# Sudo42b/vision.cpp

Measured on AMD Instinct MI355X. Metric: images/sec, Depth-Anything-V2-Small 518x518 f16, higher is better.
Workload: dtype f16; 1 GPU; Depth-Anything-V2-Small f16 (DINOv2-S ViT) 518x518 batch=32 per MI355X (BASELINE.json configs[1]); global_batch=32, weights=random-init synthetic GGUF (seed 0), parallelism=dp1 (image shards, no data-path collective), hip_graph=True

## Files before the change

### vision.cpp_amd/csrc/kernels_attn.hip

```cpp
#include "vx_common.h"

#include <cstdlib>
#include <type_traits>

namespace {

#ifndef VISP_ATTN_WPE
#define VISP_ATTN_WPE 4
#endif
#ifndef VISP_ATTN_RS
#define VISP_ATTN_RS 1
#endif
#ifndef VISP_ATTN_SEQ
#define VISP_ATTN_SEQ 1
#endif
constexpr int HD = 64;
constexpr int KV_TILE = 64;
constexpr int Q_PER_WAVE = 32;
constexpr int TILE_BYTES = KV_TILE * HD * 2;
constexpr float FAST_LIMIT_DEFAULT = 1024.0f;

typedef __fp16 hv4 __attribute__((__vector_size__(4 * sizeof(__fp16))));

__device__ __forceinline__ int v_swz(int row, int chunk16) { return chunk16 ^ (((row >> 1) & 1) << 2); }

template <int NW, bool STAMP = false>
__global__ __launch_bounds__(64 * NW) __attribute__((amdgpu_waves_per_eu(VISP_ATTN_WPE, VISP_ATTN_WPE))) void attention_kernel(const f16* __restrict__ Q, const f16* __restrict__ K,
                                                         const f16* __restrict__ V, f16* __restrict__ O, int H, int T, float FAST_LIMIT,
                                                         unsigned long long* __restrict__ stamps = nullptr) {
    unsigned long long st_wait = 0, st_soft = 0, st_pv = 0, st_t0 = 0;
    if constexpr (STAMP) st_t0 = __builtin_amdgcn_s_memtime();
    __shared__ __attribute__((aligned(16))) unsigned char smem[2 * 2 * TILE_BYTES];

    const int tid = threadIdx.x, lane = tid & 63;
    const int wave = __builtin_amdgcn_readfirstlane(tid >> 6);
    const int r = lane & 31, h = lane >> 5;
    constexpr int Q_PER_BLOCK = Q_PER_WAVE * NW;
    const int n_qblk = (T + Q_PER_BLOCK - 1) / Q_PER_BLOCK;
    int logical;
    {
        const int total = gridDim.x, id = blockIdx.x;
        const int per = total >> 3, rem = total & 7, xcd = id & 7;
        logical = (xcd < rem ? xcd * (per + 1) : rem * (per + 1) + (xcd - rem) * per) + (id >> 3);
    }
    const int bh = logical / n_qblk;
    const int q0 = (logical - bh * n_qblk) * Q_PER_BLOCK + wave * Q_PER_WAVE;

    const f16* Qb = Q + (long)bh * T * HD;
    const f16* Kb = K + (long)bh * T * HD;
    const f16* Vb = V + (long)bh * T * HD;

    f16x8 qf[4];
    {
        int qrow = q0 + r;
        if (qrow >= T) qrow = T - 1;
#pragma unroll
        for (int s = 0; s < 4; ++s) qf[s] = *reinterpret_cast<const f16x8*>(Qb + (long)qrow * HD + 16 * s + 8 * h);
    }

    const int l_row = lane >> 3, l_pos = lane & 7;
    const int n_tiles = (T + KV_TILE - 1) / KV_TILE;
    const __amdgpu_buffer_rsrc_t k_rsrc = __builtin_amdgcn_make_buffer_rsrc(const_cast<f16*>(Kb), 0, T * HD * 2, 0x00020000);
    const __amdgpu_buffer_rsrc_t v_rsrc = __builtin_amdgcn_make_buffer_rsrc(const_cast<f16*>(Vb), 0, T * HD * 2, 0x00020000);

    auto issue_loads = [&](int t, int buf) {
        unsigned char* sk = smem + buf * (2 * TILE_BYTES);
        unsigned char* sv = sk + TILE_BYTES;
        const int tile_bytes0 = t * (KV_TILE * HD * 2);
        constexpr int PER = 8 / NW;
#pragma unroll
        for (int i = 0; i < PER; ++i) {
            const int piece = wave * PER + i, row = piece * 8 + l_row;
            __builtin_amdgcn_raw_ptr_buffer_load_lds(k_rsrc, (lptr_t)(sk + piece * 1024), 16,
                                                     tile_bytes0 + row * (HD * 2) + swz128(row, l_pos) * 16, 0, 0, 0);
            __builtin_amdgcn_raw_ptr_buffer_load_lds(v_rsrc, (lptr_t)(sv + piece * 1024), 16,
                                                     tile_bytes0 + row * (HD * 2) + v_swz(row, l_pos) * 16, 0, 0, 0);
        }
    };

    f32x16 o[2];
#pragma unroll
    for (int e = 0; e < 16; ++e) { o[0][e] = 0.0f; o[1][e] = 0.0f; }
    float m_run = 0.0f;
    float l_run = 0.0f;

    const int tr_q = (lane & 15) >> 2, tr_p = lane & 3, tr_d0 = 16 * ((lane >> 4) & 1);
    const int k_off0 = r * 128 + swz128(r, h) * 16;
    int v_off0;
    {
        const int key = 4 * h + tr_q, dd = tr_d0 + 4 * tr_p;
        v_off0 = key * 128 + v_swz(key, dd >> 3) * 16 + (dd & 7) * 2;
    }
    auto k_off = [&](int st) { return k_off0 ^ (st << 5); };
    auto v_off = [&](int db) { return v_off0 ^ (db << 6); };

    f32x16 negm;
#pragma unroll
    for (int e = 0; e < 16; ++e) negm[e] = 0.0f;

    auto qk = [&](const unsigned char* sk, int kb, int k0, bool masked) {
        f32x16 s;
#pragma unroll
        for (int st = 0; st < 4; ++st) {
            f16x8 kf = *reinterpret_cast<const f16x8*>(sk + k_off(st) + kb * 4096);
            s = __builtin_amdgcn_mfma_f32_32x32x16_f16(kf, qf[st], st == 0 ? negm : s, 0, 0, 0);
        }
        if (masked) {
#pragma unroll
            for (int e = 0; e < 16; ++e) {
                const int key = k0 + kb * 32 + (e & 3) + 8 * (e >> 2) + 4 * h;
                if (key >= T) s[e] = -INFINITY;
            }
        }
        return s;
    };
    const f16x8 ones = {(f16)1, (f16)1, (f16)1, (f16)1, (f16)1, (f16)1, (f16)1, (f16)1};
    auto softmax_p = [&](const unsigned char* sk, int k0, bool masked, f16x8 (&pf)[4]) {
#pragma unroll
        for (int kb = 0; kb < 2; ++kb) {
            f32x16 s = qk(sk, kb, k0, masked);
#pragma unroll
            for (int e = 0; e < 16; ++e) pf[2 * kb + (e >> 3)][e & 7] = (f16)__builtin_amdgcn_exp2f(s[e]);
            if (VISP_ATTN_SEQ) __builtin_amdgcn_sched_barrier(0);
        }
        if constexpr (VISP_ATTN_RS) {
            typedef _Float16 h2 __attribute__((ext_vector_type(2)));
            h2 t[16];
#pragma unroll
            for (int i = 0; i < 16; ++i) t[i] = h2{pf[i >> 2][2 * (i & 3)], pf[i >> 2][2 * (i & 3) + 1]};
#pragma unroll
            for (int w = 8; w >= (VISP_ATTN_RS == 2 ? 4 : 1); w >>= 1)
#pragma unroll
                for (int i = 0; i < w; ++i) t[i] = t[i] + t[i + w];
            float half_sum;
            if (VISP_ATTN_RS == 2)
                half_sum = (((float)t[0][0] + (float)t[0][1]) + ((float)t[1][0] + (float)t[1][1])) + (((float)t[2][0] + (float)t[2][1]) + ((float)t[3][0] + (float)t[3][1]));
            else
                half_sum = (float)t[0][0] + (float)t[0][1];
            return half_sum + other_half(half_sum);
        }
        f32x16 rs = {0.f, 0.f, 0.f, 0.f, 0.f, 0.f, 0.f, 0.f, 0.f, 0.f, 0.f, 0.f, 0.f, 0.f, 0.f, 0.f};
#pragma unroll
        for (int ks = 0; ks < 4; ++ks) rs = __builtin_amdgcn_mfma_f32_32x32x16_f16(ones, pf[ks], rs, 0, 0, 0);
        return rs[0];
    };
    auto pv = [&](const unsigned char* sv, const f16x8 (&pf)[4]) {
#pragma unroll
        for (int ks = 0; ks < 4; ++ks) {
#pragma unroll
            for (int db = 0; db < 2; ++db) {
                hv4 va = __builtin_amdgcn_ds_read_tr16_b64_v4f16(
                    (__attribute__((address_space(3))) hv4*)(sv + v_off(db) + ks * 2048));
                hv4 vb = __builtin_amdgcn_ds_read_tr16_b64_v4f16(
                    (__attribute__((address_space(3))) hv4*)(sv + v_off(db) + ks * 2048 + 1024));
                f16x8 vf = {(f16)va[0], (f16)va[1], (f16)va[2], (f16)va[3], (f16)vb[0], (f16)vb[1], (f16)vb[2], (f16)vb[3]};
                o[db] = __builtin_amdgcn_mfma_f32_32x32x16_f16(vf, pf[ks], o[db], 0, 0, 0);
            }
        }
    };

    auto tile_body = [&](int t, auto buf_c) {
        constexpr int BUF = decltype(buf_c)::value;
        unsigned long long c0 = 0, c1 = 0, c2 = 0;
        if constexpr (STAMP) c0 = __builtin_amdgcn_s_memtime();
        wait_vmcnt<0>();
        __syncthreads();
        if (t + 1 < n_tiles) issue_loads(t + 1, BUF ^ 1);
        if constexpr (STAMP) { c1 = __builtin_amdgcn_s_memtime(); st_wait += c1 - c0; }
        const unsigned char* sk = smem + BUF * (2 * TILE_BYTES);
        const unsigned char* sv = sk + TILE_BYTES;
        if (q0 >= T) return;
        const int k0 = t * KV_TILE;
        const bool last = k0 + KV_TILE > T;
        f16x8 pf[4];
        float psum = 0.0f;

        bool done = false;
        if (t > 0 && !last) {
            psum = softmax_p(sk, k0, false, pf);
            done = !__any(!(psum <= FAST_LIMIT));
        }
        if (!done) {
            float mloc = -INFINITY;
#pragma unroll
            for (int kb = 0; kb < 2; ++kb) {
                const f32x16 s = qk(sk, kb, k0, last);
#pragma unroll
                for (int e = 0; e < 16; ++e) mloc = fmaxf(mloc, s[e]);
                __builtin_amdgcn_sched_barrier(0);
            }
            mloc = fmaxf(mloc, other_half(mloc));
            const float delta = t == 0 ? mloc : fmaxf(mloc, 0.0f);
            if (t == 0 || __any(delta > 0.0f)) {
                if (t > 0) {
                    const float alpha = __builtin_amdgcn_exp2f(-delta);
                    l_run *= alpha;
#pragma unroll
                    for (int e = 0; e < 16; ++e) { o[0][e] *= alpha; o[1][e] *= alpha; }
                }
                m_run += delta;
#pragma unroll
                for (int e = 0; e < 16; ++e) negm[e] = -m_run;
            }
            psum = softmax_p(sk, k0, last, pf);
        }
        l_run += psum;
        if constexpr (STAMP) { c2 = __builtin_amdgcn_s_memtime(); st_soft += c2 - c1; }
        pv(sv, pf);
        if constexpr (STAMP) {
            asm volatile("s_nop 0" ::"v"(o[0][0]), "v"(o[1][0]));
            st_pv += __builtin_amdgcn_s_memtime() - c2;
        }
    };

    issue_loads(0, 0);
    for (int t = 0; t < n_tiles; t += 2) {
        tile_body(t, std::integral_constant<int, 0>{});
        if (t + 1 < n_tiles) tile_body(t + 1, std::integral_constant<int, 1>{});
    }

    if constexpr (STAMP) {
        if (lane == 0) {
            unsigned long long* s = stamps + ((size_t)blockIdx.x * NW + wave) * 4;
            s[0] = st_wait; s[1] = st_soft; s[2] = st_pv; s[3] = __builtin_amdgcn_s_memtime() - st_t0;
        }
    }
    float inv = 1.0f / l_run;
    const int q = q0 + r;
    if (q < T) {
        const int b = bh / H, head = bh - b * H;
        f16* orow = O + ((long)b * T + q) * (H * HD) + head * HD;
#pragma unroll
        for (int db = 0; db < 2; ++db)
#pragma unroll
            for (int g = 0; g < 4; ++g) {
                f16x4 v;
#pragma unroll
                for (int j = 0; j < 4; ++j) v[j] = (f16)(o[db][g * 4 + j] * inv);
                *reinterpret_cast<f16x4*>(orow + db * 32 + 8 * g + 4 * h) = v;
            }
    }
}

}

static float g_fast_limit = FAST_LIMIT_DEFAULT;
extern "C" void vx_attention_set_fast_limit(float limit) { g_fast_limit = limit < 0.0f ? FAST_LIMIT_DEFAULT : limit; }

static void* g_attn_stamps = nullptr;
extern "C" void vx_attention_set_stamps(void* stamps) { g_attn_stamps = stamps; }

extern "C" int vx_attention_f16(const void* q, const void* k, const void* v, void* out, int B, int H, int T, void* stream) {
    VX_REQUIRE(B > 0 && H > 0 && T > 0, "vx_attention_f16: empty problem");
    static const int nw_env = getenv("VISP_ATTN_WAVES") ? atoi(getenv("VISP_ATTN_WAVES")) : 0;
    const int nw = nw_env == 4 || nw_env == 8 ? nw_env : (T > 512 ? 8 : 4);
    const int qpb = Q_PER_WAVE * nw;
    dim3 grid(((T + qpb - 1) / qpb) * B * H);
    if (g_attn_stamps)
        hipLaunchKernelGGL((nw == 8 ? attention_kernel<8, true> : attention_kernel<4, true>), grid, dim3(64 * nw), 0, as_stream(stream), reinterpret_cast<const f16*>(q),
                           reinterpret_cast<const f16*>(k), reinterpret_cast<const f16*>(v), reinterpret_cast<f16*>(out), H, T, g_fast_limit,
                           static_cast<unsigned long long*>(g_attn_stamps));
    else
        hipLaunchKernelGGL((nw == 8 ? attention_kernel<8, false> : attention_kernel<4, false>), grid, dim3(64 * nw), 0, as_stream(stream), reinterpret_cast<const f16*>(q),
                           reinterpret_cast<const f16*>(k), reinterpret_cast<const f16*>(v), reinterpret_cast<f16*>(out), H, T, g_fast_limit,
                           static_cast<unsigned long long*>(nullptr));
    VX_LAUNCH_CHECK();
    return 1;
}
```

Before: 6409 images/s.

## Pair partial query tails of two heads into one attention block

When the sequence remainder fits in half of an 8-wave block, the tail query tiles of two heads share one block. Each half of the block uses its own LDS ring and loads the K/V tiles with only its 4 waves. This removes the idle waves that tail blocks used to carry and shrinks the grid. In exchange, LDS per 8-wave block doubles and block-index mapping becomes more complex.

```diff
diff --git a/vision.cpp_amd/csrc/kernels_attn.hip b/vision.cpp_amd/csrc/kernels_attn.hip
--- a/vision.cpp_amd/csrc/kernels_attn.hip
+++ b/vision.cpp_amd/csrc/kernels_attn.hip
@@ -18,6 +18,20 @@
 constexpr int KV_TILE = 64;
 constexpr int Q_PER_WAVE = 32;
 constexpr int TILE_BYTES = KV_TILE * HD * 2;
+constexpr int RING_BYTES = 2 * 2 * TILE_BYTES;
+#ifndef VISP_ATTN_PAIR_TAILS
+#define VISP_ATTN_PAIR_TAILS 1
+#endif
+
+__host__ __device__ inline bool tail_paired(int nw, int T) {
+    const int rem = T % (Q_PER_WAVE * 8);
+    return VISP_ATTN_PAIR_TAILS && nw == 8 && rem > 0 && rem <= 4 * Q_PER_WAVE;
+}
+__host__ inline int attention_blocks(int nw, int B, int H, int T) {
+    const int qpb = Q_PER_WAVE * nw;
+    if (tail_paired(nw, T)) return (T / qpb) * B * H + (B * H + 1) / 2;
+    return ((T + qpb - 1) / qpb) * B * H;
+}
 constexpr float FAST_LIMIT_DEFAULT = 1024.0f;
 
 typedef __fp16 hv4 __attribute__((__vector_size__(4 * sizeof(__fp16))));
@@ -26,11 +40,11 @@
 
 template <int NW, bool STAMP = false>
 __global__ __launch_bounds__(64 * NW) __attribute__((amdgpu_waves_per_eu(VISP_ATTN_WPE, VISP_ATTN_WPE))) void attention_kernel(const f16* __restrict__ Q, const f16* __restrict__ K,
-                                                         const f16* __restrict__ V, f16* __restrict__ O, int H, int T, float FAST_LIMIT,
+                                                         const f16* __restrict__ V, f16* __restrict__ O, int BH, int H, int T, float FAST_LIMIT,
                                                          unsigned long long* __restrict__ stamps = nullptr) {
     unsigned long long st_wait = 0, st_soft = 0, st_pv = 0, st_t0 = 0;
     if constexpr (STAMP) st_t0 = __builtin_amdgcn_s_memtime();
-    __shared__ __attribute__((aligned(16))) unsigned char smem[2 * 2 * TILE_BYTES];
+    __shared__ __attribute__((aligned(16))) unsigned char smem[(NW == 8 ? 2 : 1) * RING_BYTES];
 
     const int tid = threadIdx.x, lane = tid & 63;
     const int wave = __builtin_amdgcn_readfirstlane(tid >> 6);
@@ -43,8 +57,32 @@
         const int per = total >> 3, rem = total & 7, xcd = id & 7;
         logical = (xcd < rem ? xcd * (per + 1) : rem * (per + 1) + (xcd - rem) * per) + (id >> 3);
     }
-    const int bh = logical / n_qblk;
-    const int q0 = (logical - bh * n_qblk) * Q_PER_BLOCK + wave * Q_PER_WAVE;
+    int bh = logical / n_qblk;
+    int q0 = (logical - bh * n_qblk) * Q_PER_BLOCK + wave * Q_PER_WAVE;
+    int ring_off = 0, piece0 = wave * (8 / NW), n_piece = 8 / NW;
+    if constexpr (NW == 8) {
+        if (tail_paired(NW, T)) {
+            const int n_full = T / Q_PER_BLOCK, grp = 2 * n_full + 1;
+            const int pair = logical / grp, idx = logical - pair * grp;
+            if (idx == n_full) {
+                const int half = wave >> 2, w = wave & 3;
+                bh = 2 * pair + half;
+                q0 = n_full * Q_PER_BLOCK + w * Q_PER_WAVE;
+                ring_off = half * RING_BYTES;
+                piece0 = 2 * w;
+                n_piece = 2;
+                if (bh >= BH) {
+                    bh = BH - 1;
+                    q0 = T;
+                    n_piece = 0;
+                }
+            } else {
+                const int second = idx > n_full;
+                bh = 2 * pair + second;
+                q0 = (idx - second * (n_full + 1)) * Q_PER_BLOCK + wave * Q_PER_WAVE;
+            }
+        }
+    }
 
     const f16* Qb = Q + (long)bh * T * HD;
     const f16* Kb = K + (long)bh * T * HD;
@@ -64,13 +102,14 @@
     const __amdgpu_buffer_rsrc_t v_rsrc = __builtin_amdgcn_make_buffer_rsrc(const_cast<f16*>(Vb), 0, T * HD * 2, 0x00020000);
 
     auto issue_loads = [&](int t, int buf) {
-        unsigned char* sk = smem + buf * (2 * TILE_BYTES);
+        unsigned char* sk = smem + ring_off + buf * (2 * TILE_BYTES);
         unsigned char* sv = sk + TILE_BYTES;
         const int tile_bytes0 = t * (KV_TILE * HD * 2);
-        constexpr int PER = 8 / NW;
+        constexpr int PER = NW == 8 ? 2 : 8 / NW;
 #pragma unroll
         for (int i = 0; i < PER; ++i) {
-            const int piece = wave * PER + i, row = piece * 8 + l_row;
+            if (NW == 8 && i >= n_piece) break;
+            const int piece = piece0 + i, row = piece * 8 + l_row;
             __builtin_amdgcn_raw_ptr_buffer_load_lds(k_rsrc, (lptr_t)(sk + piece * 1024), 16,
                                                      tile_bytes0 + row * (HD * 2) + swz128(row, l_pos) * 16, 0, 0, 0);
             __builtin_amdgcn_raw_ptr_buffer_load_lds(v_rsrc, (lptr_t)(sv + piece * 1024), 16,
@@ -85,11 +124,11 @@
     float l_run = 0.0f;
 
     const int tr_q = (lane & 15) >> 2, tr_p = lane & 3, tr_d0 = 16 * ((lane >> 4) & 1);
-    const int k_off0 = r * 128 + swz128(r, h) * 16;
+    const int k_off0 = ring_off + r * 128 + swz128(r, h) * 16;
     int v_off0;
     {
         const int key = 4 * h + tr_q, dd = tr_d0 + 4 * tr_p;
-        v_off0 = key * 128 + v_swz(key, dd >> 3) * 16 + (dd & 7) * 2;
+        v_off0 = ring_off + key * 128 + v_swz(key, dd >> 3) * 16 + (dd & 7) * 2;
     }
     auto k_off = [&](int st) { return k_off0 ^ (st << 5); };
     auto v_off = [&](int db) { return v_off0 ^ (db << 6); };
@@ -254,15 +293,14 @@
     VX_REQUIRE(B > 0 && H > 0 && T > 0, "vx_attention_f16: empty problem");
     static const int nw_env = getenv("VISP_ATTN_WAVES") ? atoi(getenv("VISP_ATTN_WAVES")) : 0;
     const int nw = nw_env == 4 || nw_env == 8 ? nw_env : (T > 512 ? 8 : 4);
-    const int qpb = Q_PER_WAVE * nw;
-    dim3 grid(((T + qpb - 1) / qpb) * B * H);
+    dim3 grid(attention_blocks(nw, B, H, T));
     if (g_attn_stamps)
         hipLaunchKernelGGL((nw == 8 ? attention_kernel<8, true> : attention_kernel<4, true>), grid, dim3(64 * nw), 0, as_stream(stream), reinterpret_cast<const f16*>(q),
-                           reinterpret_cast<const f16*>(k), reinterpret_cast<const f16*>(v), reinterpret_cast<f16*>(out), H, T, g_fast_limit,
+                           reinterpret_cast<const f16*>(k), reinterpret_cast<const f16*>(v), reinterpret_cast<f16*>(out), B * H, H, T, g_fast_limit,
                            static_cast<unsigned long long*>(g_attn_stamps));
     else
         hipLaunchKernelGGL((nw == 8 ? attention_kernel<8, false> : attention_kernel<4, false>), grid, dim3(64 * nw), 0, as_stream(stream), reinterpret_cast<const f16*>(q),
-                           reinterpret_cast<const f16*>(k), reinterpret_cast<const f16*>(v), reinterpret_cast<f16*>(out), H, T, g_fast_limit,
+                           reinterpret_cast<const f16*>(k), reinterpret_cast<const f16*>(v), reinterpret_cast<f16*>(out), B * H, H, T, g_fast_limit,
                            static_cast<unsigned long long*>(nullptr));
     VX_LAUNCH_CHECK();
     return 1;
```

Result: no change. 6397 images/s (-0.2%).
